# OSUrobotics/KinovaGrasping

Measured on AMD Instinct MI355X. Metric: env-steps/sec (whole node) at 4096 envs/GPU, higher is better.
Workload: dtype f32

## Files before the change

### include/kinova_sim.h

```cpp
#ifndef KINOVA_SIM_H
#define KINOVA_SIM_H
#include <stddef.h>
#include <stdint.h>

#ifdef __cplusplus
extern "C" {
#endif

#define KS_NQ 16
#define KS_NV 15
#define KS_NACT 4
#define KS_NOBS 82
#define KS_NINFO 3
#define KS_NCON_MAX 24
#define KS_NCON_MAX_MG 40
#define KS_CONTACT_STRIDE 20

typedef enum {
    KS_OK = 0,
    KS_ERR_INVALID = -1,
    KS_ERR_NO_DEVICE = -2,
    KS_ERR_HIP = -3,
    KS_ERR_MODEL = -4,
    KS_ERR_STATE = -5
// ... 49 lines not shown
int ks_set_env_params(ks_ctx *ctx, const void *obj_mass, const void *obj_mu, void *stream);

int ks_set_param_ranges(ks_ctx *ctx, const void *ranges, uint64_t seed, void *stream);
int ks_get_env_params(ks_ctx *ctx, void *mass, void *mu, int64_t *episode, void *stream);

int ks_substep(ks_ctx *ctx, const void *ctrl, void *stream);

int ks_obs_from_snapshot(ks_ctx *ctx, const void *snap, const void *rays, void *obs, void *reward, uint8_t *done, void *info, void *stream);

typedef struct {
    const float *actor_pub;
    const int64_t *actor_ver;
    int64_t actor_stride;
    int64_t off_w1, off_b1, off_w2, off_b2, off_w3, off_b3;
    int32_t h1, h2;
    float sigma, max_action;
    int32_t skip_steps;
    int32_t with_replay;
    uint64_t seed;
    float *obs, *prev_obs;
    uint8_t *has_prev, *ready, *lifting;
    int64_t *t, *steps_total;
    float *action, *action_t;
    float *reward_out; uint8_t *done_out;
    void *sim_obs, *sim_reward; uint8_t *sim_done; void *sim_info, *sim_final_obs;
    int32_t horizon, n_steps;
    float *cur_state, *cur_next, *cur_action, *cur_reward, *cur_not_done;
    int64_t *cur_len;
    uint8_t *cur_sel;
    int64_t *pub_len;
    int64_t *counters;
    int64_t budget_ticks;
    int64_t *repeats;
} ks_rollout_args;
int ks_rollout(ks_ctx *ctx, int32_t n_iter, const ks_rollout_args *args_host, void *stream);

enum { KS_CONTROLLER_NONE = 0, KS_CONTROLLER_NAIVE = 1, KS_CONTROLLER_POSITION_DEPENDENT = 2, KS_CONTROLLER_COMBINED = 3 };
enum { KS_LIFT_RULE_TRAIN = 0, KS_LIFT_RULE_EXPERT = 1 };
int ks_set_rollout_controller(ks_ctx *ctx, int32_t mode, int32_t lift_rule, void *stream);
int ks_get_rollout_controller(ks_ctx *ctx, int32_t *mode, int32_t *lift_rule, float *init, void *stream);

enum { KS_PLAN_WAVES = 0, KS_PLAN_WORKGROUPS = 1, KS_PLAN_QUEUE = 2, KS_PLAN_RUNS = 3, KS_PLAN_ROUND_ROBIN = 4 };
int ks_rollout_plan(ks_ctx *ctx, int32_t *mode, int32_t *groups, int32_t *workgroups);

int ks_kernel_time(ks_ctx *ctx, int reset, double *avg_ms_host, int64_t *launches_host);

int ks_version(void);

#ifdef __cplusplus
}
#endif
#endif
```

### kinovagrasping_amd/build.py

```python
from __future__ import annotations

import os
import shutil
import subprocess
from pathlib import Path

PKG = Path(__file__).resolve().parent
CSRC = PKG / "csrc"
LIB = PKG / "libkinova_sim.so"
LIB_MG = PKG / "libkinova_sim_mg.so"
SOURCES = ["ks_api.hip", "ks_rollout.hip", "ks_mlp.hip", "ks_xchg.hip"]
HEADERS = ["ks_math.h", "ks_model.h", "ks_model_host.h", "ks_core.h", "ks_obs.h", "ks_env.h", "ks_mlp_tile.h", "../../include/kinova_sim.h", "../../include/kinova_rollout.h"]


def hipcc_path() -> str:
    for cand in (os.environ.get("HIPCC"), shutil.which("hipcc"), "/opt/rocm/bin/hipcc"):
        if cand and Path(cand).exists():
            return cand
    raise RuntimeError("hipcc not found (need ROCm; this package has no CPU build)")


def needs_build(lib: Path = LIB) -> bool:
    if not lib.exists():
        return True
    t = lib.stat().st_mtime
    return any((CSRC / f).stat().st_mtime > t for f in SOURCES + HEADERS)


def build(force: bool = False, verbose: bool = False, multi_geom: bool | None = None) -> Path:
    for mg in ([False, True] if multi_geom is None else [bool(multi_geom)]):
        lib = LIB_MG if mg else LIB
        if not force and not needs_build(lib):
            continue
        cmd = [hipcc_path(), "--offload-arch=gfx950", "-O3", "-std=c++17", "-fPIC", "-shared"] + (["-DKS_MULTI_GEOM"] if mg else []) + \
              ["-o", str(lib)] + [str(CSRC / s) for s in SOURCES]
        if verbose:
            cmd.insert(1, "-Rpass-analysis=kernel-resource-usage")
        subprocess.check_call(cmd, cwd=str(CSRC))
    return LIB_MG if multi_geom else LIB
```

### kinovagrasping_amd/csrc/ks_api.hip

```cpp
#include <hip/hip_runtime.h>

#include <algorithm>
#include <cstdio>
#include <cstdlib>
#include <cstring>
#include <type_traits>
#include <map>
#include <string>
#include <vector>

#include "../../include/kinova_sim.h"
#include "ks_env.h"
#include "ks_mlp_tile.h"
#include "ks_select.h"
#include "ks_model_host.h"

using namespace ks;

namespace {

constexpr int WAVE = 64;
thread_local std::string g_create_error;

template <typename T> struct StartPool {
    int32_t k, pad;
    uint64_t seed;
    const T *qpos0, *hand_quat, *obs0;
    T *env_qpos0, *env_hand_quat, *env_obs0;
    int64_t *episode;
    int32_t *index;
};

template <typename T> struct EpisodeLog {
    int32_t capacity, pad;
    unsigned long long *written;
    ks_episode_record *ring;
    int32_t *ordinal;
    const int32_t *obj_id;
    const T *obs0;
    const StartPool<T> *pool;
};

template <typename T> struct ParamRanges {
    int32_t active, pad;
    uint64_t seed;
    const T *ranges;
    T *envp;
// ... 757 lines not shown
    kmlp::f32x4(*H1)[NR] = (kmlp::f32x4(*)[NR])(float*)wblocks;
    kmlp::f32x4(*H2)[NR] = H1 + NT1 * 4;
    kmlp::f32x4(*X)[NR] = H2 + NT2 * 4;
    const int lane = threadIdx.x & 63;
    for (;;) {
        const long long ver = uniform64(__hip_atomic_load(ra.actor_ver, __ATOMIC_RELAXED, __HIP_MEMORY_SCOPE_AGENT));
        __builtin_amdgcn_fence(__ATOMIC_ACQUIRE, "agent");
        const float* pw = ra.actor_pub + (ver % 3) * ra.actor_stride;
        kmlp::f32x4 z4 = {0.f, 0.f, 0.f, 0.f};
        int ln = lane, rw = row_env;
        asm volatile("" : "+v"(ln), "+v"(rw));
        const bool mine = kmlp::mlp3_rows_wave<NT1, NT2, true, NR>(ln, (long)rw, S, ra.h1, ra.h2, A, ra.obs, S, kmlp::x_bytes(N, 0, S, S), pw + ra.off_w1,
                                                                     pw + ra.off_b1, pw + ra.off_w2, pw + ra.off_b2, pw + ra.off_w3, X, H1, H2, z4);
        float y[4] = {0.f, 0.f, 0.f, 0.f};
        if (mine) policy_squash(ra, z4, pw + ra.off_b3, y);
        __builtin_amdgcn_fence(__ATOMIC_ACQUIRE, "agent");
        const long long ver2 = uniform64(__hip_atomic_load(ra.actor_ver, __ATOMIC_RELAXED, __HIP_MEMORY_SCOPE_AGENT));
        if (ver2 - ver < 2) {
            if (mine) policy_select(ra, N, row_env, y);
            return;
        }
        if (lane == 0 && ra.repeats) atomicAdd((unsigned long long*)ra.repeats, 1ull);
    }
}

#ifdef KS_ROLLOUT_STAMP
#define KS_RS(i) { const long long t1_ = wall_clock64(); if (C::tid() == 0) atomicAdd((unsigned long long*)&rap->counters[4 + i], (unsigned long long)(t1_ - tk)); tk = t1_; }
#else
#define KS_RS(i)
#endif
template <int NT1, int NT2, bool WAVE_SCOPE>
__device__ __forceinline__ void rollout_iter(const Model<float>& m, const Hulls<float>& hu, const Buffers<float>* __restrict__ bdev, int N, int frame_skip,
                                             int iters, int epw, int pair_memory, const ObsOut<float>* __restrict__ out,
                                             const ks_rollout_args* __restrict__ rap, KS_LDS float* blocks, int grp) {
    using T = float;
    using C = Crew<WAVE_SCOPE>;
    const Buffers<T>& b = *bdev;
    const int e = threadIdx.x / LANE_STRIDE;
    const Team<SUBS> team{(int)threadIdx.x % LANE_STRIDE};
    const int env = e < epw ? b.slot_env[grp * epw + e] : -1;
    const bool active = !(team.sub >= SUBS || env < 0);
    const int wave = WAVE_SCOPE ? (int)(threadIdx.x >> 6) : 0;
    const int slot0 = grp * epw + 4 * wave, cepw = WAVE_SCOPE ? (epw - 4 * wave < 4 ? (epw - 4 * wave < 0 ? 0 : epw - 4 * wave) : 4) : epw;
    KS_LDS T* cblocks = blocks + 4 * wave * SCR_TOTAL;
    KS_LDS unsigned* w = (KS_LDS unsigned*)cblocks;
    const auto join = [] {
        if constexpr (!WAVE_SCOPE) __threadfence_block();
        C::sync();
    };
#ifdef KS_ROLLOUT_STAMP
    long long tk = wall_clock64();
#endif
    {
        const int nn = C::tid() & 15;
        const int row_env = nn < cepw ? b.slot_env[slot0 + nn] : -1;
        if (b.ctl->mode != 0) rollout_controller(b.ctl, rap, N, C::tid() < 16 ? row_env : -1);
        else if constexpr (WAVE_SCOPE) rollout_policy_wave<NT1, NT2>(rap, N, row_env, cblocks);
        else rollout_policy<NT1, NT2>(rap, N, row_env, cblocks);
    }
    join();
    KS_RS(0)
    if (active) {
        T hq[4], act[4];
        KS_UNROLL
        for (int i = 0; i < 4; i++) { hq[i] = b.hand_quat[(long)i * N + env]; act[i] = rap->action_t[(long)i * N + env]; }
        int ncon = 0, status = 0;
        ColW<T> snap{b.snap + env, N};
        KS_LDS T* blk = blocks + e * SCR_TOTAL;
        ScratchC<T, KS_LDS T*> scr{blk};
        T* stp = (T*)(blk + SCR_STATE);
        load_state_team<T, SUBS>(b, env, N, stp, team.sub);
        load_env_params(scr, team, b, env, N);
        constexpr int WPL = (NPAIR_MAX + SUBS - 1) / SUBS;
        PairWarm gw[WPL];
        unsigned* pm = b.pairmem + ((long)env * SUBS + team.sub) * (WPL * WARM_WORDS);
        KS_UNROLL
// ... 25 lines not shown
    if (active) rollout_store<float>(rap, N, env, team.sub);
    join();
    KS_RS(3)
}
#undef KS_RS

struct GroupDeal {
    int n, g0, g1, gstep;
    __device__ __forceinline__ explicit GroupDeal(int n_groups) {
        const bool rr = n_groups < 0;
        n = rr ? -n_groups : n_groups;
        g0 = rr ? (int)blockIdx.x : (int)((long)blockIdx.x * n / gridDim.x);
        g1 = rr ? n : (int)((long)(blockIdx.x + 1) * n / gridDim.x);
        gstep = rr ? (int)gridDim.x : 1;
    }
    __device__ __forceinline__ bool several() const { return g1 - g0 > gstep; }
};
__device__ __forceinline__ bool object_differs(const int32_t* wg_model, int grp, int& staged) {
    const int want = __builtin_amdgcn_readfirstlane(wg_model[grp]);
    if (want == staged) return false;
    staged = want;
    return true;
}

__device__ __noinline__ int rollout_restage(const Model<float>* __restrict__ mp, KS_LDS float* lds0, Hulls<float>* hup) {
    __syncthreads();
    const Model<float>* ml = stage_model_and_tables<float, WG>(mp, lds0);
    int hull_words = 0;
    __syncthreads();
    stage_hulls<float, true>(*ml, lds0 + model_words<float>(), hull_words, *hup, true);
    return (hull_words >> 2) << 2;
}

template <int NT1, int NT2>
__global__ __launch_bounds__(WG) KS_ROLLOUT_REGS void k_rollout(const Model<float>* __restrict__ models, Buffers<float> b, const Buffers<float>* __restrict__ bdev, int N,
                                                int frame_skip, int iters, int epw, int pair_memory, const ObsOut<float>* __restrict__ out,
                                                const ks_rollout_args* __restrict__ rap, int n_iter, int n_groups, int* __restrict__ queue, int wave_free) {
    using T = float;
    extern __shared__ __attribute__((aligned(16))) unsigned char smem[];
#ifdef KS_ROLLOUT_STAMP
    const long long wk_entry = wall_clock64();
#endif
    const GroupDeal deal(n_groups);
    KS_LDS T* const lds0 = (KS_LDS T*)smem;
    KS_LDS T* const lds = lds0 + model_words<T>();
    Hulls<T>* const hup = (Hulls<T>*)(smem + (sizeof(Model<T>) + 15) / 16 * 16);
    int staged = __builtin_amdgcn_readfirstlane(b.wg_model[deal.g0]);
    const Model<T>* ml = stage_model_and_tables<T, WG>(models + staged, lds0);
    int hull_words = 0;
    __syncthreads();
    stage_hulls<T, true>(*ml, lds, hull_words, *hup, true);
    KS_LDS T* blocks = env_blocks(lds, hull_words);
#ifdef KS_ROLLOUT_STAMP
    const long long wk_loop = wall_clock64();
    const long long ck_loop = clock64();
#endif
#define KS_STEP_GROUP(WAVE_SCOPE, GRP)                                                                                      \
    const Model<T>* mi = ml;                                                                                                \
    Hulls<T>* hi = hup;                                                                                                     \
    const Buffers<T>* bi = bdev;                                                                                            \
    const ObsOut<T>* oi = out;                                                                                              \
    const ks_rollout_args* ri = rap;                                                                                        \
    KS_LDS T* ki = blocks;                                                                                                  \
    int gi = GRP;                                                                                                           \
    asm volatile("" : "+s"(mi), "+s"(hi), "+s"(bi), "+s"(oi), "+s"(ri), "+s"(gi));                                          \
    asm volatile("" : "+v"(ki));                                                                                            \
    rollout_iter<NT1, NT2, WAVE_SCOPE>(*mi, *hi, bi, N, frame_skip, iters, epw, pair_memory, oi, ri, ki, gi)
    if (wave_free) {
        const long long budget = rap->budget_ticks, t_end = wall_clock64() + budget;
#pragma clang loop unroll(disable)
        for (int it = 0; it < n_iter; it++) {
            if (budget > 0 && it > 0 && wall_clock64() - t_end > 0) break;
            KS_STEP_GROUP(true, deal.g0);
        }
        return;
    }
    if (queue != nullptr) {
        __shared__ int s_grp;
        int* const q_head = queue, * const q_tail = queue + 1, * const q_steps = queue + ROLLOUT_Q_STEPS;
        unsigned* const ring = (unsigned*)(queue + ROLLOUT_Q_RING);
        const int total = deal.n * n_iter;
#pragma clang loop unroll(disable)
        for (;;) {
            __syncthreads();
            if (threadIdx.x == 0) {
                const int t = atomicAdd(q_head, 1);
                int grp = -1;
                if (t < total) {
                    const unsigned lap = (unsigned)(t / ROLLOUT_QCAP) + 1u;
                    unsigned v = __hip_atomic_load(&ring[t % ROLLOUT_QCAP], __ATOMIC_ACQUIRE, __HIP_MEMORY_SCOPE_AGENT);
                    while ((v >> 12) != lap) {
                        __builtin_amdgcn_s_sleep(16);
                        v = __hip_atomic_load(&ring[t % ROLLOUT_QCAP], __ATOMIC_ACQUIRE, __HIP_MEMORY_SCOPE_AGENT);
                    }
                    grp = (int)(v & 4095u) - 1;
                }
                s_grp = grp;
            }
            __syncthreads();
            const int grp = __builtin_amdgcn_readfirstlane(s_grp);
            if (grp < 0) break;
            __builtin_amdgcn_fence(__ATOMIC_ACQUIRE, "agent");
            if (object_differs(bdev->wg_model, grp, staged)) blocks = lds + rollout_restage(models + staged, lds0, hup);
            KS_STEP_GROUP(false, grp);
            __builtin_amdgcn_fence(__ATOMIC_RELEASE, "agent");
            __syncthreads();
            if (threadIdx.x == 0) {
                const int c = q_steps[gi] + 1;
                q_steps[gi] = c;
                if (c < n_iter) {
                    __builtin_amdgcn_fence(__ATOMIC_RELEASE, "agent");
                    const int t2 = atomicAdd(q_tail, 1);
                    __hip_atomic_store(&ring[t2 % ROLLOUT_QCAP], (((unsigned)(t2 / ROLLOUT_QCAP) + 1u) << 12) | (unsigned)(gi + 1), __ATOMIC_RELEASE, __HIP_MEMORY_SCOPE_AGENT);
                }
            }
        }
        return;
    }
#pragma clang loop unroll(disable)
    for (int it = 0; it < n_iter; it++) {
#pragma clang loop unroll(disable)
        for (int grp = deal.g0; grp < deal.g1; grp += deal.gstep) {
            if (deal.several() && object_differs(bdev->wg_model, grp, staged)) blocks = lds + rollout_restage(models + staged, lds0, hup);
            KS_STEP_GROUP(false, grp);
        }
    }
#undef KS_STEP_GROUP
#ifdef KS_ROLLOUT_STAMP
    if (threadIdx.x == 0 && blockIdx.x < 512) {
        const long long wk_end = wall_clock64();
        rap->counters[8 + blockIdx.x] = wk_entry;
        rap->counters[8 + 512 + blockIdx.x] = wk_loop - wk_entry;
        rap->counters[8 + 1024 + blockIdx.x] = wk_end - wk_loop;
        rap->counters[8 + 1536 + blockIdx.x] = clock64() - ck_loop;
    }
#endif
}

template <typename T, bool USE_LDS>
__global__ __launch_bounds__(WG) void k_substep(const Model<T>* __restrict__ models, Buffers<T> b, const T* __restrict__ ctrl, int N, int iters, int epw, int tap) {
    extern __shared__ __attribute__((aligned(16))) unsigned char smem[];
    KS_LDS T* lds = (KS_LDS T*)smem;
    const Model<T>* mp = models + b.wg_model[blockIdx.x];
    const Model<T>* ml = mp;
    if constexpr (USE_LDS) { ml = stage_model(mp, lds); lds += model_words<T>(); }
    const Model<T>& m = *ml;
    int hull_words = 0;
    static_assert(sizeof(Hulls<T>) <= HULLS_BYTES, "Hulls descriptor slot");
    Hulls<T> hu_own;
    Hulls<T>* hup = &hu_own;
    if constexpr (USE_LDS) hup = (Hulls<T>*)(smem + (sizeof(Model<T>) + 15) / 16 * 16);
    stage_hulls<T, USE_LDS>(*mp, lds, hull_words, *hup);
    const Hulls<T>& hu = *hup;
    const int e = threadIdx.x / LANE_STRIDE;
    const Team<SUBS> team{(int)threadIdx.x % LANE_STRIDE};
    const int env = e < epw ? b.slot_env[blockIdx.x * epw + e] : -1;
    if (team.sub >= SUBS || env < 0) return;
// ... 766 lines not shown
        HIPCHK(hipMemcpy(d_model, table.data(), sizeof(Model<T>) * nm, hipMemcpyHostToDevice));
        if ((r = alloc(&b.nominal, nominal.size()))) return r;
        HIPCHK(hipMemcpy(b.nominal, nominal.data(), nominal.size() * sizeof(T), hipMemcpyHostToDevice));
        {
            std::vector<T> ep(2 * (size_t)cfg.n_envs, nominal[1]);
            std::fill(ep.begin(), ep.begin() + cfg.n_envs, nominal[0]);
            HIPCHK(hipMemcpy(b.envp, ep.data(), ep.size() * sizeof(T), hipMemcpyHostToDevice));
        }
        if ((r = plan_launch()) != KS_OK) return r;
        n_wg = (cfg.n_envs + lpw - 1) / lpw + (nm - 1);
        if ((r = alloc(&b.slot_env, (size_t)n_wg * lpw))) return r;
        if ((r = alloc(&b.wg_model, (size_t)n_wg))) return r;
        if ((r = alloc(&b.n_used, (size_t)1))) return r;
        if ((r = alloc(&b.rayq, (size_t)4 + 2 * (size_t)n_wg))) return r;
        if (obs_in_step && cfg.frame_skip >= 1 && !(getenv("KS_RAY_POOL") && getenv("KS_RAY_POOL")[0] == '0')) {
            ray_pool = 2;
        }
        if ((r = regroup(0, true))) return r;
        if ((r = alloc(&d_b, (size_t)1))) return r;
        if ((r = alloc(&d_out, (size_t)1))) return r;
        if (!h_out) HIPCHK(hipHostMalloc((void**)&h_out, (H_OUT_RING + CAPTURE_RECORDS) * sizeof(ObsOut<T>), hipHostMallocDefault));
        if (!d_ra) HIPCHK(hipMalloc((void**)&d_ra, sizeof(ks_rollout_args)));
        if (!d_queue) HIPCHK(hipMalloc((void**)&d_queue, ROLLOUT_Q_WORDS * sizeof(int)));
        if (!h_ra) HIPCHK(hipHostMalloc((void**)&h_ra, sizeof(ks_rollout_args) * (H_OUT_RING + CAPTURE_RECORDS), hipHostMallocDefault));
        HIPCHK(hipMemcpy(d_b, &b, sizeof b, hipMemcpyHostToDevice));
        model_loaded = true;
        return KS_OK;
    }
    int blocks() const { return (cfg.n_envs + WAVE - 1) / WAVE; }
    int resident_wgs = 256;
    int* d_queue = nullptr;
    bool rollout_queue = !MULTI_GEOM;
    bool rollout_waves = !(getenv("KS_ROLLOUT_WAVES") && getenv("KS_ROLLOUT_WAVES")[0] == '0');
    int rollout_phase_deal = getenv("KS_ROLLOUT_PHASE_DEAL") ? atoi(getenv("KS_ROLLOUT_PHASE_DEAL")) : 1;
    bool rollout_round_robin = false;
    int lpw = WAVE;
    bool rays_in_step = false, obs_in_step = false;
    int ray_pool = 0;
    size_t step_lds = 0;
    int hull_words = 0;
    int plan_launch() {
        {
            int cus = 0;
            if (hipDeviceGetAttribute(&cus, hipDeviceAttributeMultiprocessorCount, device) != hipSuccess || cus <= 0) cus = 256;
            if (const char* e = getenv("KS_ROLLOUT_WGS")) { const int v = atoi(e); if (v > 0) cus = v; }
            resident_wgs = cus;
            rollout_round_robin = n_models > 1;
            if (const char* e = getenv("KS_ROLLOUT_DEAL")) { rollout_round_robin = strcmp(e, "rr") == 0; rollout_queue = strcmp(e, "queue") == 0; }
        }
        const size_t lds_max = 160 * 1024;
        const size_t hull_bytes = (size_t)hull_words * sizeof(T) + (USE_LDS ? (size_t)model_words<T>() * sizeof(T) : 0);
        const size_t per_env = USE_LDS ? (size_t)SCR_TOTAL * sizeof(T) : 0;
        int cap = USE_LDS ? (int)((lds_max - hull_bytes - 64) / per_env) : EPW_MAX;
        if (cap > EPW_MAX) cap = EPW_MAX;
        if (cap < 1) { error = "hull tables do not fit in LDS"; return KS_ERR_MODEL; }
        int want = cfg.envs_per_wave > 0 ? cfg.envs_per_wave : EPW_MAX;
        lpw = want > cap ? cap : want;
        step_lds = hull_bytes + per_env * lpw;
        rays_in_step = USE_LDS && sizeof(T) == 4 && (size_t)wg_rays_words(lpw) <= (size_t)SCR_TOTAL * lpw &&
                       !(getenv("KS_RAYS_IN_STEP") && getenv("KS_RAYS_IN_STEP")[0] == '0');
        obs_in_step = rays_in_step && (size_t)(wg_rays_words(EPW_MAX) + wg_obs_words(EPW_MAX) + 4) <= (size_t)SCR_TOTAL * lpw &&
                      !(getenv("KS_OBS_IN_STEP") && getenv("KS_OBS_IN_STEP")[0] == '0');
        if (getenv("KS_DEBUG")) fprintf(stderr, "[ks] stepping kernel: %d envs per workgroup, LDS %zu B (tables %zu B, %zu B per env), limit %zu\n", lpw, step_lds, hull_bytes, per_env, lds_max);
        HIPCHK(hipFuncSetAttribute((const void*)step_kernel(), hipFuncAttributeMaxDynamicSharedMemorySize, (int)step_lds));
        HIPCHK(hipFuncSetAttribute((const void*)k_substep<T, USE_LDS>, hipFuncAttributeMaxDynamicSharedMemorySize, (int)step_lds));
        return KS_OK;
    }
    static constexpr auto step_kernel() {
        if constexpr (sizeof(T) == 4) return &k_env_step_f32;
        else return &k_env_step<T, USE_LDS>;
    }
    ObsOut<T> out_record(void* obs, void* reward, uint8_t* done, void* info, void* final_obs) const {
        return ObsOut<T>{(T*)obs, (T*)reward, done, (T*)info, (T*)final_obs, cfg.horizon, cfg.auto_reset, cfg.obs_env_major};
    }
    int regroup(hipStream_t s, bool loading = false) {
        hipLaunchKernelGGL(k_slots, dim3(1), dim3(SLOT_THREADS), 0, s, b.obj_id, cfg.n_envs, n_models, lpw, n_wg, b.slot_env, b.wg_model, b.n_used);
        if (loading) {
            HIPCHK(hipGetLastError());
            HIPCHK(hipDeviceSynchronize());
        } else if (stream_is_capturing(s)) { n_groups = n_wg; return KS_OK; }
        HIPCHK(hipMemcpyAsync(&n_groups, b.n_used, sizeof(int32_t), hipMemcpyDeviceToHost, s));
        HIPCHK(hipStreamSynchronize(s));
        return KS_OK;
    }
    void clear_pool(hipStream_t s) {
// ... 140 lines not shown
                                  lpw, (const ObsOut<T>*)d_out, (const ks_rollout_args*)d_ra, n_iter, rollout_round_robin ? -n_groups : n_groups,
                                  (int)ws_offset);
        });
#endif
    }
    int rollout(int n_iter, const ks_rollout_args* ra, hipStream_t s) override {
        if (int r = need_model("ks_rollout")) return r;
        if constexpr (sizeof(T) != 4) return rollout_exact(n_iter, ra, s);
        else {
            int r;
            if ((r = check_rollout_buffers(n_iter, ra))) return r;
            if (!obs_in_step || !cfg.obs_env_major || !cfg.auto_reset) { error = "ks_rollout needs the in-kernel observation path, env-major observations and auto_reset"; return KS_ERR_STATE; }
            if ((r = check_rollout_actor(ra))) return r;
            if (policy_lds_bytes(ra->h1, ra->h2) > (size_t)SCR_TOTAL * lpw * sizeof(T)) { error = "ks_rollout: no LDS for the policy"; return KS_ERR_STATE; }
            const int N = cfg.n_envs;
            const bool wave_free = plan_waves() && policy_wave_lds_bytes(ra->h1, ra->h2) <= (size_t)SCR_TOTAL * 4 * sizeof(T);
            if (ra->budget_ticks != 0 && (ra->budget_ticks < 0 || !wave_free)) {
                error = "ks_rollout: a time budget needs the wave form of the rollout kernel (ks_rollout_plan: KS_PLAN_WAVES)";
                return KS_ERR_STATE;
            }
            if ((r = send_rollout_records(ra, s))) return r;
            const bool use_queue = plan_queue();
            if (use_queue) {
                hipLaunchKernelGGL(k_rollout_queue_init, dim3(1), dim3(256), 0, s, d_queue, n_groups);
            }
            if (wave_free && rollout_phase_deal != 0 && n_models == 1 && ra->budget_ticks == 0) {
                if (rollout_phase_deal == 2 && N <= PHASE_ENVS_MAX) hipLaunchKernelGGL(k_slots_by_phase, dim3(1), dim3(PHASE_THREADS), 0, s, (const int64_t*)ra->t, N, n_wg * lpw, b.slot_env);
                else if (lpw <= 16) hipLaunchKernelGGL(k_slots_by_phase_in_groups, dim3((n_groups + 255) / 256), dim3(256), 0, s, (const int64_t*)ra->t, n_groups, lpw, b.slot_env);
            }
            return launch_for_widths(ra, [&](auto tiles) {
                using W = decltype(tiles);
                return launch_rollout(k_rollout<W::NT1, W::NT2>, step_lds, s, d_model, b, (const Buffers<T>*)d_b, N, cfg.frame_skip, cfg.solver_iterations, lpw,
                                      (int)cfg.pair_memory, (const ObsOut<T>*)d_out, (const ks_rollout_args*)d_ra, n_iter,
                                      (use_queue || !rollout_round_robin) ? n_groups : -n_groups, use_queue ? d_queue : (int*)nullptr, (int)wave_free);
            });
        }
    }
    bool plan_queue() const { return rollout_queue && n_groups > resident_wgs && n_groups <= ROLLOUT_QCAP; }
    bool plan_waves() const {
        return rollout_waves && !plan_queue() && n_groups <= resident_wgs && lpw == EPW_MAX && LANE_STRIDE == SUBS &&
               (size_t)(wg_rays_words(4, WAVE) + wg_obs_words(4) + 4) <= (size_t)SCR_TOTAL * 4;
    }
    int rollout_plan(int32_t* mode, int32_t* groups, int32_t* workgroups) override {
        if (int r = need_model("ks_rollout_plan")) return r;
        if constexpr (sizeof(T) != 4) {
            if (mode) *mode = n_groups <= resident_wgs ? KS_PLAN_WORKGROUPS : (rollout_round_robin ? KS_PLAN_ROUND_ROBIN : KS_PLAN_RUNS);
        } else if (mode) *mode = plan_waves() ? KS_PLAN_WAVES : (n_groups <= resident_wgs ? KS_PLAN_WORKGROUPS : (plan_queue() ? KS_PLAN_QUEUE : (rollout_round_robin ? KS_PLAN_ROUND_ROBIN : KS_PLAN_RUNS)));
        if (groups) *groups = n_groups;
        if (workgroups) *workgroups = n_groups < resident_wgs ? n_groups : resident_wgs;
        return KS_OK;
    }
    int set_start_pool(int k, const void* q0, const void* hq, uint64_t seed, void* obs, hipStream_t s) override {
        if (int r = need_model("ks_set_start_pool")) return r;
        if (k == 0) {
            clear_pool(s);
            HIPCHK(hipGetLastError());
            return KS_OK;
        }
        if (k < 1 || k > POOL_K_MAX || !q0 || !hq) { error = "ks_set_start_pool: 1 <= k <= 1024 starts per env (0 clears the pool), qpos0 and hand_quat required"; return KS_ERR_INVALID; }
        const size_t N = cfg.n_envs;
        int r;
        if (!pb.snap) {
            Buffers<T> t = b;
            if ((r = alloc(&t.qpos, NQ * N))) return r;
            if ((r = alloc(&t.qvel, NV * N))) return r;
            if ((r = alloc(&t.warm, NV * N))) return r;
            if ((r = alloc(&t.rays, NRAY * N))) return r;
// ... 312 lines not shown
```

### kinovagrasping_amd/pipeline.py

```python
from __future__ import annotations

import os
from functools import partial

import torch


def _concurrent_stream(main, dev, tries=8):
    import time
    import warnings
    torch.cuda.synchronize(dev)
    e0, e1 = torch.cuda.Event(enable_timing=True), torch.cuda.Event(enable_timing=True)
    with torch.cuda.stream(main):
        e0.record(main)
        torch.cuda._sleep(1000000)
        e1.record(main)
    torch.cuda.synchronize(dev)
    ms = max(1e-3, e0.elapsed_time(e1))
    spin = int(1000000 * min(1e4, 25.0 / ms))
    flag = torch.zeros(1, device=dev)
    cand = None
    for _ in range(tries):
        cand = torch.cuda.Stream(dev)
        ev = torch.cuda.Event()
# ... 295 lines not shown
                        for _ in range(self.updates_per_step - 1):
                            self.g_head.replay()
                            self._body()
                main.wait_event(self.head_done)
        elif learn:
            for _ in range(self.updates_per_step):
                self.g_head.replay()
                self._body()
        if self.direct_post:
            self.eng.post(commit=False)
        else:
            self.g_post.replay()
        self.pending_commit = self.defer_commit
        self.steps += 1
        return self.eng.reward_out, self.eng.done_out

    def _commit_pending(self):
        if self.pending_commit:
            self.g_commit.replay()
            self.pending_commit = False

    def flush(self, finish_update=False):
        if self.pending_commit or finish_update:
            self.side.wait_stream(self.main)
            with torch.cuda.stream(self.side):
                self._commit_pending()
                if finish_update:
                    self.native.finish_pending()
            self.main.wait_stream(self.side)
        if self.distributed and self.native.exchange is not None:
            self.native.exchange.check()


def rollout_args(sim, policy, eng, pub, pub_ver, steps_total, counters, replay=None, repeats=None, sigma=None):
    from .rollout import SKIP_NUM_TS
    from .sim import KsRolloutArgs
    P = lambda t: t.data_ptr()
    a = KsRolloutArgs()
    if getattr(eng, "controller", None) is None or policy is not None:
        flat, actor = policy._flat_params["actor"], policy.actor
        off = lambda t: (t.data_ptr() - flat.data_ptr()) // 4
        a.actor_pub, a.actor_ver, a.actor_stride = P(pub), P(pub_ver), pub.shape[1]
        a.off_w1, a.off_b1, a.off_w2, a.off_b2, a.off_w3, a.off_b3 = (off(actor.l1.weight), off(actor.l1.bias), off(actor.l2.weight), off(actor.l2.bias),
                                                                      off(actor.l3.weight), off(actor.l3.bias))
        a.h1, a.h2 = actor.l1.weight.shape[0], actor.l2.weight.shape[0]
    a.sigma, a.max_action, a.skip_steps, a.with_replay, a.seed = (eng.sigma if sigma is None else sigma), eng.max_action, SKIP_NUM_TS, int(replay is not None), eng.noise_seed
    a.obs, a.prev_obs, a.has_prev, a.ready, a.lifting = P(eng.obs), P(eng.prev_obs), P(eng.has_prev), P(eng.ready), P(eng.lifting)
    a.t, a.steps_total, a.action, a.action_t = P(eng.t), P(steps_total), P(eng.action), P(eng.action_t)
    a.reward_out, a.done_out = P(eng.reward_out), P(eng.done_out)
    a.sim_obs, a.sim_reward, a.sim_done, a.sim_info, a.sim_final_obs = P(sim.obs), P(sim.reward), P(sim.done), P(sim.info), P(sim.final_obs)
    if replay is not None:
        a.horizon, a.n_steps = replay.horizon, replay.n_steps
        a.cur_state, a.cur_next, a.cur_action = P(replay.a_state), P(replay.a_next), P(replay.a_action)
        a.cur_reward, a.cur_not_done, a.cur_len = P(replay.a_reward), P(replay.a_not_done), P(replay.a_len)
        a.cur_sel, a.pub_len = P(replay.a_sel), P(replay.pub_len)
    a.counters = P(counters)
    if repeats is not None:
        a.repeats = P(repeats)
    return a


class AsyncTrainer(GraphedTrainer):

    def __init__(self, sim, policy, replay, engine, batch_episodes=64, expert_replay=None, expert_prob=0.3, updates_per_step=1,
                 launch_synchronous=False, max_launch_steps=60, balanced=False, prioritized=False, per_alpha=0.3, per_beta=1.0, per_eps=1e-3,
                 per_eps_expert=1.0, tables=None):
        if prioritized and launch_synchronous:
            raise ValueError("AsyncTrainer: launch_synchronous stages episodes in a ring without priorities - not with prioritized=True")
        super().__init__(sim, policy, replay, engine, batch_episodes=batch_episodes, overlap=True, expert_replay=expert_replay, expert_prob=expert_prob,
                         updates_per_step=updates_per_step, lean_learner="auto", balanced=balanced, prioritized=prioritized, per_alpha=per_alpha,
                         per_beta=per_beta, per_eps=per_eps, per_eps_expert=per_eps_expert, tables=tables)
        self.launch_synchronous = bool(launch_synchronous)
        if self.launch_synchronous and getattr(replay, "ep_class", None) is not None:
            raise ValueError("AsyncTrainer: launch_synchronous stages episodes in a ring without classes - not with a replay that has classes set")
        if self.launch_synchronous:
            from .replay import DeviceEpisodeReplay
            self.stage = DeviceEpisodeReplay(replay.n_envs, capacity=(max(1, int(max_launch_steps)) // 10 + 2) * replay.n_envs, horizon=replay.horizon, state_dim=replay.ep_state.shape[2],
                                             action_dim=replay.ep_action.shape[2], n_steps=replay.n_steps, device=replay.device)
            self._stage_rank = torch.zeros(self.stage.capacity, dtype=torch.long, device=replay.device)
            self._stage_pos = torch.arange(1, self.stage.capacity + 1, dtype=torch.long, device=replay.device)
            g = torch.Generator(device="cpu").manual_seed(0)
            self._key_w = (torch.rand(replay.horizon * replay.ep_action.shape[2], generator=g, dtype=torch.float64).to(replay.device),
                           torch.rand(replay.ep_state.shape[2], generator=g, dtype=torch.float64).to(replay.device))
        eng, dev = engine, self.dev
        if not self.native.lds_free:
            raise ValueError("AsyncTrainer needs the LDS-free learner kernels (hidden widths 256-256 / 128-128 / 64-64, or the lean ones: 400-300): the persistent rollout kernel "
                             "holds every CU's LDS for the whole launch, a learner built on library GEMMs could only run behind it")
        self.replica_sync = "per-update" if self.distributed else "single rank"
        self.library_allreduce_chunk = None
        if self.distributed and self.native.exchange is None:
            import torch.distributed as dist
            forced = os.environ.get("KS_ASYNC_SYNC", "")
            if forced == "average":
                import warnings
                warnings.warn("AsyncTrainer: KS_ASYNC_SYNC=average - replicas apply LOCAL updates and are averaged at every launch boundary (periodic model "
                              "averaging), not north_star's per-update gradient all-reduce", RuntimeWarning)
                self.replica_sync = "average-per-launch"
                self.native.local_gradients = True
                self.exchange_note += "; free-running rollout kept: local updates, replicas averaged at every launch boundary"
            elif dist.get_backend(policy.process_group) == "nccl":
                self.library_allreduce_chunk = int(os.environ.get("KS_ASYNC_LIBRARY_CHUNK", "6"))
                self.exchange_note += (f"; no peer mapping: per-update library all-reduce, which executes between launches - keep launches at <= "
                                       f"{self.library_allreduce_chunk} env-steps (the learner lags by at most one launch)")
        if not (eng.native and eng.device_noise and eng._fused_actor_layers() is not None and sim.cfg.auto_reset and sim.obs_env_major):
            raise ValueError("AsyncTrainer needs the fused actor path (3-layer MLP at a supported width, in-kernel noise), auto_reset and env-major obs")
        flat = policy.acting_flat()
        self.actor_flat = flat
        stride = (flat.numel() + 3) // 4 * 4
        self.pub = torch.zeros(3, stride, device=dev)
        self.pub_ver = torch.zeros(1, dtype=torch.long, device=dev)
        self.n_pub = 0
        self.pub[0, :flat.numel()].copy_(flat)
        replay.enable_async()
        self.steps_total = torch.zeros(eng.n, dtype=torch.long, device=dev)
        self.counters = torch.zeros(8 + 4 * 512 + 8 + (eng.n if os.environ.get("KS_DEBUG_DROPS") else 0), dtype=torch.long, device=dev)
        self.repeats = torch.zeros(1, dtype=torch.long, device=dev)
        a = rollout_args(sim, policy, eng, self.pub, self.pub_ver, self.steps_total, self.counters, replay=replay, repeats=self.repeats)
        from .sim import load_library
        self._lib = load_library()
        self.check_in_body = False
        self.pace_lead = int(os.environ.get("KS_ASYNC_LEAD", "8"))
        self.pace_timeouts = torch.zeros(1, dtype=torch.long, device=dev)
        self.args = a
        self.env_steps = 0
        self.rollout_plan, n_groups, n_wgs = sim.rollout_plan()
        self.groups_per_workgroup = (n_groups + n_wgs - 1) // n_wgs
        if self.rollout_plan in ("runs", "round-robin") and n_groups % n_wgs:
            import warnings
            warnings.warn(f"AsyncTrainer: {n_groups} env groups dealt to {n_wgs} persistent workgroups ({self.rollout_plan}): some step {self.groups_per_workgroup} groups per "
                          f"env-step, others {self.groups_per_workgroup - 1} - the launch runs at the pace of the former (the ready queue, KS_ROLLOUT_DEAL=queue, and "
                          "GraphedTrainer's lock-step launches balance such a batch dynamically)", RuntimeWarning)

    def _stage_published(self):
        self.replay.commit_published(into=self.stage)

    def _launch_boundary(self):
        self.g_boundary.replay()
        self.publish()

    def _boundary_commit(self):
        r, st_ = self.replay, self.stage
        self._stage_published()
        cap = st_.capacity
        valid = torch.arange(cap, device=st_.device) < st_._count
        key = (st_.ep_action[:cap].reshape(cap, -1).double() * self._key_w[0]).sum(1) + (st_.ep_state[:cap, 0].double() * self._key_w[1]).sum(1) \
            + st_.ep_len[:cap].double() * 1e-3
        key = torch.where(valid, key, torch.full_like(key, float("inf")))
        order = torch.sort(key, stable=True).indices
        self._stage_rank.scatter_(0, order, self._stage_pos)
        skip = (st_._count - r.capacity).clamp(min=0)
# ... 119 lines not shown
        bufs = [pol._flat_params[k] for k in self._network_names()]
        bufs += [b for net in self._opt_nets() for b in (net.exp_avg, net.exp_avg_sq)]
        flat = torch.cat([b.reshape(-1) for b in bufs])
        dist.all_reduce(flat, op=dist.ReduceOp.SUM, group=pol.process_group)
        flat.div_(world)
        off = 0
        for b in bufs:
            b.copy_(flat[off:off + b.numel()].view_as(b))
            off += b.numel()
        if not self.launch_synchronous:
            self.publish()

    def step(self):
        self.run(1)
        return self.eng.reward_out, self.eng.done_out

    def flush(self, finish_update=False):
        self.side.wait_stream(self.main)
        with torch.cuda.stream(self.side):
            if self.launch_synchronous:
                self._launch_boundary()
            else:
                self.g_commit.replay() if self.g_commit is not None else self.replay.commit_published()
            if finish_update:
                self.native.finish_pending()
                self.publish()
        self.main.wait_stream(self.side)
        if self.distributed and self.native.exchange is not None:
            self.native.exchange.check()

    def repeated_forwards(self) -> int:
        return int(self.repeats.item())

    def counts(self):
        c = self.counters[:4].tolist()
        return {"episodes_finished": c[0], "lifted": c[1], "episodes_kept": c[2], "episodes_dropped": c[3], "pacing_timeouts": int(self.pace_timeouts.item())}
```

### kinovagrasping_amd/sim.py

```python
from __future__ import annotations

import ctypes as C
from pathlib import Path

import torch

from . import build as _build

NQ, NV, NACT, NOBS, NINFO, NCON_MAX, CONTACT_STRIDE = 16, 15, 4, 82, 3, 24, 20
NCON_MAX_MG = 40
SOLVER_ITERATIONS = 20
ASSETS = Path(__file__).resolve().parent / "assets"


class KsConfig(C.Structure):
    _fields_ = [("n_envs", C.c_int32), ("frame_skip", C.c_int32), ("horizon", C.c_int32), ("solver_iterations", C.c_int32),
                ("precision", C.c_int32), ("auto_reset", C.c_int32), ("obs_env_major", C.c_int32), ("envs_per_wave", C.c_int32),
                ("contact_tap", C.c_int32), ("pair_memory", C.c_int32), ("reserved", C.c_int32 * 2)]


class KrRing(C.Structure):
    _fields_ = [("count", C.c_void_p), ("head", C.c_void_p), ("capacity", C.c_int32), ("ep_len", C.c_void_p), ("ep_state", C.c_void_p),
                ("ep_next", C.c_void_p), ("ep_action", C.c_void_p), ("ep_reward", C.c_void_p), ("ep_not_done", C.c_void_p)]


class KsRolloutArgs(C.Structure):
    _fields_ = ([("actor_pub", C.c_void_p), ("actor_ver", C.c_void_p), ("actor_stride", C.c_int64)] +
                [(k, C.c_int64) for k in ("off_w1", "off_b1", "off_w2", "off_b2", "off_w3", "off_b3")] +
                [("h1", C.c_int32), ("h2", C.c_int32), ("sigma", C.c_float), ("max_action", C.c_float), ("skip_steps", C.c_int32),
                 ("with_replay", C.c_int32), ("seed", C.c_uint64)] +
                [(k, C.c_void_p) for k in ("obs", "prev_obs", "has_prev", "ready", "lifting", "t", "steps_total", "action", "action_t", "reward_out",
                                           "done_out", "sim_obs", "sim_reward", "sim_done", "sim_info", "sim_final_obs")] +
                [("horizon", C.c_int32), ("n_steps", C.c_int32)] +
                [(k, C.c_void_p) for k in ("cur_state", "cur_next", "cur_action", "cur_reward", "cur_not_done", "cur_len", "cur_sel", "pub_len", "counters")] +
                [("budget_ticks", C.c_int64), ("repeats", C.c_void_p)])


class KsEpisodeRecord(C.Structure):
    _fields_ = [("env", C.c_int32), ("object", C.c_int32), ("start_index", C.c_int32), ("steps", C.c_int32), ("done", C.c_int32),
                ("start_x", C.c_float), ("start_y", C.c_float), ("episode", C.c_int32)]


EPISODE_RECORD_WORDS = 8
CONTROLLER_MODES = {None: 0, "naive": 1, "position-dependent": 2, "combined": 3}
LIFT_RULES = {"train": 0, "expert": 1}


def controller_codes(mode, lift_rule):
    if mode not in CONTROLLER_MODES or lift_rule not in LIFT_RULES:
        raise ValueError(f"controller {mode!r} / lift rule {lift_rule!r}: one of {[m for m in CONTROLLER_MODES if m]} (or None) and one of {list(LIFT_RULES)}")
    return CONTROLLER_MODES[mode], LIFT_RULES[lift_rule]

EPISODE_LOG_CAPACITY_MAX = 1 << 24


def decode_episode_ring(ring: torch.Tensor, written: int, cursor: int, capacity: int):
    written, cursor, capacity = int(written), int(cursor), int(capacity)
    if tuple(ring.shape) != (capacity, EPISODE_RECORD_WORDS) or ring.dtype != torch.int32:
        raise ValueError("decode_episode_ring: ring int32 [capacity, 8]")
    if not 0 <= cursor <= written:
        raise ValueError("decode_episode_ring: 0 <= cursor <= written")
    first = max(cursor, written - capacity)
    tickets = torch.arange(first, written, dtype=torch.long, device=ring.device)
    return ring[tickets % capacity], first - cursor


def episode_records(words: torch.Tensor) -> dict:
    words = words.contiguous()
# ... 389 lines not shown
```

Before: 2.938 million.

## Add intra-workgroup wave work-stealing takeover for wave-free rollout

Adds an LDS-based protocol that lets a wave that has finished its own iterations request half of another wave's env slots in the same workgroup and keep stepping them. The aim is to cut idle tail time when waves in a workgroup finish unevenly, keeping CUs busy until all env slots finish their iterations. In exchange each iteration adds a small state-machine step with LDS atomics, a noinline call and possible spin-sleeps. It runs by default when the budget is zero, and adds takeover counters to the rollout args.

```diff
diff --git a/include/kinova_sim.h b/include/kinova_sim.h
--- a/include/kinova_sim.h
+++ b/include/kinova_sim.h
@@ -105,6 +105,7 @@
     int64_t *counters;
     int64_t budget_ticks;
     int64_t *repeats;
+    int64_t *takeovers;
 } ks_rollout_args;
 int ks_rollout(ks_ctx *ctx, int32_t n_iter, const ks_rollout_args *args_host, void *stream);
 
diff --git a/kinovagrasping_amd/build.py b/kinovagrasping_amd/build.py
--- a/kinovagrasping_amd/build.py
+++ b/kinovagrasping_amd/build.py
@@ -10,7 +10,7 @@
 LIB = PKG / "libkinova_sim.so"
 LIB_MG = PKG / "libkinova_sim_mg.so"
 SOURCES = ["ks_api.hip", "ks_rollout.hip", "ks_mlp.hip", "ks_xchg.hip"]
-HEADERS = ["ks_math.h", "ks_model.h", "ks_model_host.h", "ks_core.h", "ks_obs.h", "ks_env.h", "ks_mlp_tile.h", "../../include/kinova_sim.h", "../../include/kinova_rollout.h"]
+HEADERS = ["ks_math.h", "ks_model.h", "ks_model_host.h", "ks_core.h", "ks_obs.h", "ks_env.h", "ks_mlp_tile.h", "ks_select.h", "ks_controller.h", "ks_takeover.h", "../../include/kinova_sim.h", "../../include/kinova_rollout.h"]
 
 
 def hipcc_path() -> str:
diff --git a/kinovagrasping_amd/csrc/ks_api.hip b/kinovagrasping_amd/csrc/ks_api.hip
--- a/kinovagrasping_amd/csrc/ks_api.hip
+++ b/kinovagrasping_amd/csrc/ks_api.hip
@@ -13,6 +13,7 @@
 #include "ks_env.h"
 #include "ks_mlp_tile.h"
 #include "ks_select.h"
+#include "ks_takeover.h"
 #include "ks_model_host.h"
 
 using namespace ks;
@@ -836,16 +837,17 @@
 template <int NT1, int NT2, bool WAVE_SCOPE>
 __device__ __forceinline__ void rollout_iter(const Model<float>& m, const Hulls<float>& hu, const Buffers<float>* __restrict__ bdev, int N, int frame_skip,
                                              int iters, int epw, int pair_memory, const ObsOut<float>* __restrict__ out,
-                                             const ks_rollout_args* __restrict__ rap, KS_LDS float* blocks, int grp) {
+                                             const ks_rollout_args* __restrict__ rap, KS_LDS float* blocks, int grp, int sbase, int cnt) {
     using T = float;
     using C = Crew<WAVE_SCOPE>;
     const Buffers<T>& b = *bdev;
     const int e = threadIdx.x / LANE_STRIDE;
     const Team<SUBS> team{(int)threadIdx.x % LANE_STRIDE};
-    const int env = e < epw ? b.slot_env[grp * epw + e] : -1;
+    const int wteam = (int)(threadIdx.x & (WAVE - 1)) >> 4;
+    const int env = WAVE_SCOPE ? (wteam < cnt ? b.slot_env[sbase + wteam] : -1) : (e < epw ? b.slot_env[grp * epw + e] : -1);
     const bool active = !(team.sub >= SUBS || env < 0);
     const int wave = WAVE_SCOPE ? (int)(threadIdx.x >> 6) : 0;
-    const int slot0 = grp * epw + 4 * wave, cepw = WAVE_SCOPE ? (epw - 4 * wave < 4 ? (epw - 4 * wave < 0 ? 0 : epw - 4 * wave) : 4) : epw;
+    const int slot0 = WAVE_SCOPE ? sbase : grp * epw, cepw = WAVE_SCOPE ? cnt : epw;
     KS_LDS T* cblocks = blocks + 4 * wave * SCR_TOTAL;
     KS_LDS unsigned* w = (KS_LDS unsigned*)cblocks;
     const auto join = [] {
@@ -937,6 +939,38 @@
     return (hull_words >> 2) << 2;
 }
 
+struct TakeoverLds {
+    KS_LDS uint32_t* w;
+    __device__ __forceinline__ uint32_t load(int i) { return __hip_atomic_load(w + i, __ATOMIC_RELAXED, __HIP_MEMORY_SCOPE_WORKGROUP); }
+    __device__ __forceinline__ void store(int i, uint32_t v) { __hip_atomic_store(w + i, v, __ATOMIC_RELAXED, __HIP_MEMORY_SCOPE_WORKGROUP); }
+    __device__ __forceinline__ bool cas(int i, uint32_t expect, uint32_t v) {
+        return __hip_atomic_compare_exchange_strong(w + i, &expect, v, __ATOMIC_RELAXED, __ATOMIC_RELAXED, __HIP_MEMORY_SCOPE_WORKGROUP);
+    }
+    __device__ __forceinline__ void release() { __builtin_amdgcn_fence(__ATOMIC_RELEASE, "agent"); }
+    __device__ __forceinline__ void acquire() { __builtin_amdgcn_fence(__ATOMIC_ACQUIRE, "agent"); }
+    __device__ __forceinline__ int64_t deadline_ticks() const { return 5000000; }
+};
+__device__ __noinline__ uint32_t rollout_takeover_next(uint32_t run, KS_LDS uint32_t* words, const ks_rollout_args* __restrict__ rap) {
+    uint32_t next = 0u;
+    if ((threadIdx.x & (WAVE - 1)) == 0) {
+        TakeoverLds mem{words};
+        kstk::Wave w = kstk::resume((int)(threadIdx.x >> 6), run);
+        for (;;) {
+            w.idle = 0;
+            const kstk::Event ev = kstk::advance(w, mem, (int64_t)wall_clock64());
+            if (ev == kstk::STEP) { next = kstk::pack_run(w.off, w.cnt, w.left); break; }
+            if (ev == kstk::EXIT) break;
+            if (w.idle) __builtin_amdgcn_s_sleep(64);
+        }
+        if (int64_t* tk = rap->takeovers) {
+            if (w.grants) atomicAdd((unsigned long long*)&tk[0], (unsigned long long)w.grants);
+            if (w.expiries) atomicAdd((unsigned long long*)&tk[1], (unsigned long long)w.expiries);
+            if (w.grants_from_pairs) atomicAdd((unsigned long long*)&tk[2], (unsigned long long)w.grants_from_pairs);
+        }
+    }
+    return (uint32_t)__builtin_amdgcn_readfirstlane((int)next);
+}
+
 template <int NT1, int NT2>
 __global__ __launch_bounds__(WG) KS_ROLLOUT_REGS void k_rollout(const Model<float>* __restrict__ models, Buffers<float> b, const Buffers<float>* __restrict__ bdev, int N,
                                                 int frame_skip, int iters, int epw, int pair_memory, const ObsOut<float>* __restrict__ out,
@@ -953,6 +987,8 @@
     int staged = __builtin_amdgcn_readfirstlane(b.wg_model[deal.g0]);
     const Model<T>* ml = stage_model_and_tables<T, WG>(models + staged, lds0);
     int hull_words = 0;
+    __shared__ uint32_t s_tko[kstk::WORDS];
+    if (wave_free == 2 && threadIdx.x < kstk::WORDS) s_tko[threadIdx.x] = kstk::initial_word((int)threadIdx.x, epw, n_iter);
     __syncthreads();
     stage_hulls<T, true>(*ml, lds, hull_words, *hup, true);
     KS_LDS T* blocks = env_blocks(lds, hull_words);
@@ -960,23 +996,28 @@
     const long long wk_loop = wall_clock64();
     const long long ck_loop = clock64();
 #endif
-#define KS_STEP_GROUP(WAVE_SCOPE, GRP)                                                                                      \
+#define KS_STEP_GROUP(WAVE_SCOPE, GRP, SBASE, CNT)                                                                          \
     const Model<T>* mi = ml;                                                                                                \
     Hulls<T>* hi = hup;                                                                                                     \
     const Buffers<T>* bi = bdev;                                                                                            \
     const ObsOut<T>* oi = out;                                                                                              \
     const ks_rollout_args* ri = rap;                                                                                        \
     KS_LDS T* ki = blocks;                                                                                                  \
-    int gi = GRP;                                                                                                           \
-    asm volatile("" : "+s"(mi), "+s"(hi), "+s"(bi), "+s"(oi), "+s"(ri), "+s"(gi));                                          \
+    int gi = GRP, si = SBASE, ci = CNT;                                                                                     \
+    asm volatile("" : "+s"(mi), "+s"(hi), "+s"(bi), "+s"(oi), "+s"(ri), "+s"(gi), "+s"(si), "+s"(ci));                      \
     asm volatile("" : "+v"(ki));                                                                                            \
-    rollout_iter<NT1, NT2, WAVE_SCOPE>(*mi, *hi, bi, N, frame_skip, iters, epw, pair_memory, oi, ri, ki, gi)
+    rollout_iter<NT1, NT2, WAVE_SCOPE>(*mi, *hi, bi, N, frame_skip, iters, epw, pair_memory, oi, ri, ki, gi, si, ci)
     if (wave_free) {
         const long long budget = rap->budget_ticks, t_end = wall_clock64() + budget;
+        const int wave = __builtin_amdgcn_readfirstlane((int)(threadIdx.x >> 6));
+        uint32_t run = kstk::pack_run(4 * wave, kstk::initial_cnt(wave, epw), wave_free == 2 ? n_iter + 1 : n_iter);
 #pragma clang loop unroll(disable)
-        for (int it = 0; it < n_iter; it++) {
-            if (budget > 0 && it > 0 && wall_clock64() - t_end > 0) break;
-            KS_STEP_GROUP(true, deal.g0);
+        for (int it = 0;; it++) {
+            if (wave_free == 2) {
+                run = (uint32_t)__builtin_amdgcn_readfirstlane((int)rollout_takeover_next(run, (KS_LDS uint32_t*)s_tko, rap));
+                if (run == 0u) break;
+            } else if (it >= n_iter || (budget > 0 && it > 0 && wall_clock64() - t_end > 0)) break;
+            KS_STEP_GROUP(true, deal.g0, __builtin_amdgcn_readfirstlane(deal.g0 * epw + kstk::run_off(run)), __builtin_amdgcn_readfirstlane(kstk::run_cnt(run)));
         }
         return;
     }
@@ -1007,7 +1048,7 @@
             if (grp < 0) break;
             __builtin_amdgcn_fence(__ATOMIC_ACQUIRE, "agent");
             if (object_differs(bdev->wg_model, grp, staged)) blocks = lds + rollout_restage(models + staged, lds0, hup);
-            KS_STEP_GROUP(false, grp);
+            KS_STEP_GROUP(false, grp, 0, 0);
             __builtin_amdgcn_fence(__ATOMIC_RELEASE, "agent");
             __syncthreads();
             if (threadIdx.x == 0) {
@@ -1027,7 +1068,7 @@
 #pragma clang loop unroll(disable)
         for (int grp = deal.g0; grp < deal.g1; grp += deal.gstep) {
             if (deal.several() && object_differs(bdev->wg_model, grp, staged)) blocks = lds + rollout_restage(models + staged, lds0, hup);
-            KS_STEP_GROUP(false, grp);
+            KS_STEP_GROUP(false, grp, 0, 0);
         }
     }
 #undef KS_STEP_GROUP
@@ -1860,6 +1901,7 @@
     int* d_queue = nullptr;
     bool rollout_queue = !MULTI_GEOM;
     bool rollout_waves = !(getenv("KS_ROLLOUT_WAVES") && getenv("KS_ROLLOUT_WAVES")[0] == '0');
+    bool rollout_takeover = !(getenv("KS_ROLLOUT_TAKEOVER") && getenv("KS_ROLLOUT_TAKEOVER")[0] == '0');
     int rollout_phase_deal = getenv("KS_ROLLOUT_PHASE_DEAL") ? atoi(getenv("KS_ROLLOUT_PHASE_DEAL")) : 1;
     bool rollout_round_robin = false;
     int lpw = WAVE;
@@ -1879,6 +1921,7 @@
         const size_t lds_max = 160 * 1024;
         const size_t hull_bytes = (size_t)hull_words * sizeof(T) + (USE_LDS ? (size_t)model_words<T>() * sizeof(T) : 0);
         const size_t per_env = USE_LDS ? (size_t)SCR_TOTAL * sizeof(T) : 0;
+        static_assert(16 + kstk::WORDS * sizeof(uint32_t) <= 64, "k_rollout's static LDS");
         int cap = USE_LDS ? (int)((lds_max - hull_bytes - 64) / per_env) : EPW_MAX;
         if (cap > EPW_MAX) cap = EPW_MAX;
         if (cap < 1) { error = "hull tables do not fit in LDS"; return KS_ERR_MODEL; }
@@ -2085,7 +2128,8 @@
                 using W = decltype(tiles);
                 return launch_rollout(k_rollout<W::NT1, W::NT2>, step_lds, s, d_model, b, (const Buffers<T>*)d_b, N, cfg.frame_skip, cfg.solver_iterations, lpw,
                                       (int)cfg.pair_memory, (const ObsOut<T>*)d_out, (const ks_rollout_args*)d_ra, n_iter,
-                                      (use_queue || !rollout_round_robin) ? n_groups : -n_groups, use_queue ? d_queue : (int*)nullptr, (int)wave_free);
+                                      (use_queue || !rollout_round_robin) ? n_groups : -n_groups, use_queue ? d_queue : (int*)nullptr,
+                                      wave_free ? ((rollout_takeover && ra->budget_ticks == 0 && n_iter < kstk::LEFT_MAX) ? 2 : 1) : 0);
             });
         }
     }
diff --git a/kinovagrasping_amd/csrc/ks_takeover.h b/kinovagrasping_amd/csrc/ks_takeover.h
--- /dev/null
+++ b/kinovagrasping_amd/csrc/ks_takeover.h
@@ -0,0 +1,154 @@
+#pragma once
+#if defined(__HIPCC__)
+#include <hip/hip_runtime.h>
+#define KTK_HD __host__ __device__ __forceinline__
+#else
+#define KTK_HD inline
+#endif
+#include <stdint.h>
+
+#ifndef KS_TAKEOVER_MIN_LEFT
+#define KS_TAKEOVER_MIN_LEFT 2
+#endif
+
+namespace kstk {
+
+constexpr int WAVES = 4, MIN_LEFT = KS_TAKEOVER_MIN_LEFT;
+constexpr int REQ = 0, PROG = WAVES, GRANT = 2 * WAVES, WORDS = 3 * WAVES;
+constexpr int LEFT_MAX = (1 << 22) - 1;
+constexpr uint32_t GRANT_BIT = 0x80000000u, DECLINED = 0x40000000u, FROM_PAIR = 0x20000000u;
+
+KTK_HD uint32_t pack_prog(int left, int cnt) { return (uint32_t)left << 3 | (uint32_t)cnt; }
+KTK_HD uint32_t pack_run(int off, int cnt, int left) { return (uint32_t)left << 7 | (uint32_t)off << 3 | (uint32_t)cnt; }
+KTK_HD int run_cnt(uint32_t r) { return (int)(r & 7u); }
+KTK_HD int run_off(uint32_t r) { return (int)(r >> 3 & 15u); }
+KTK_HD int run_left(uint32_t r) { return (int)(r >> 7 & (uint32_t)LEFT_MAX); }
+
+enum State : int {
+    W_ITER_DONE, W_CHECK, W_CLAIM, W_ANSWER, W_PUBLISH,
+    H_START, H_SCAN, H_REQUEST, H_WAIT, H_WAIT_TARGET, H_WITHDRAW, H_WAIT_ANSWER, H_TAKE, EXITED
+};
+enum Event : int { NONE, STEP, EXIT };
+
+struct Wave {
+    int me, state;
+    int off, cnt, left;
+    int q;
+    int target, k;
+    int best, best_left, best_cnt, blocked;
+    uint32_t got, prog;
+    int64_t deadline;
+    int expired;
+    int idle;
+    int grants, grants_from_pairs, expiries;
+};
+
+KTK_HD Wave resume(int me, uint32_t run) {
+    Wave w{};
+    w.me = me; w.off = run_off(run); w.cnt = run_cnt(run); w.left = run_left(run);
+    w.state = W_ITER_DONE;
+    return w;
+}
+KTK_HD int initial_cnt(int w, int epw) { return epw - 4 * w < 4 ? (epw - 4 * w < 0 ? 0 : epw - 4 * w) : 4; }
+KTK_HD uint32_t initial_word(int word, int epw, int n_iter) {
+    return (word >= PROG && word < PROG + WAVES) ? pack_prog(n_iter, initial_cnt(word - PROG, epw)) : 0u;
+}
+
+template <class M>
+KTK_HD Event advance(Wave& w, M& mem, int64_t now) {
+    switch (w.state) {
+    case W_ITER_DONE:
+        w.left--;
+        mem.store(PROG + w.me, pack_prog(w.left, w.cnt));
+        w.state = (w.left > 0 && w.cnt > 0) ? W_CHECK : H_START;
+        return NONE;
+    case W_CHECK:
+        w.q = (int)mem.load(REQ + w.me);
+        if (w.q == 0) { w.state = W_ITER_DONE; return STEP; }
+        w.state = W_CLAIM;
+        return NONE;
+    case W_CLAIM:
+        if (!mem.cas(REQ + w.me, (uint32_t)w.q, 0u)) { w.state = W_ITER_DONE; return STEP; }
+        w.state = W_ANSWER;
+        return NONE;
+    case W_ANSWER:
+        if (w.cnt >= 2 && w.left >= MIN_LEFT) {
+            const int give = w.cnt / 2;
+            mem.release();
+            mem.store(GRANT + w.q - 1, GRANT_BIT | pack_run(w.off + w.cnt - give, give, w.left) | (w.cnt == 2 ? FROM_PAIR : 0u));
+            w.cnt -= give;
+            w.state = W_PUBLISH;
+            return NONE;
+        }
+        mem.store(GRANT + w.q - 1, DECLINED);
+        w.state = W_ITER_DONE;
+        return STEP;
+    case W_PUBLISH:
+        mem.store(PROG + w.me, pack_prog(w.left, w.cnt));
+        w.state = W_ITER_DONE;
+        return STEP;
+    case H_START:
+        w.deadline = now + mem.deadline_ticks();
+        w.k = 0; w.best = -1; w.blocked = 0;
+        w.state = H_SCAN;
+        return NONE;
+    case H_SCAN: {
+        const int s = (w.me + 1 + w.k / 2) % WAVES;
+        if ((w.k & 1) == 0) w.prog = mem.load(PROG + s);
+        else {
+            const int left = (int)(w.prog >> 3), cnt = (int)(w.prog & 7u);
+            const bool pending = mem.load(REQ + s) != 0u;
+            if (cnt >= 2 && left > MIN_LEFT) {
+                if (pending) w.blocked = 1;
+                else if (w.best < 0 || left > w.best_left || (left == w.best_left && (cnt > w.best_cnt || (cnt == w.best_cnt && s < w.best)))) {
+                    w.best = s; w.best_left = left; w.best_cnt = cnt;
+                }
+            }
+        }
+        if (++w.k < 2 * (WAVES - 1)) return NONE;
+        if (w.best >= 0) { w.target = w.best; w.state = H_REQUEST; return NONE; }
+        if (w.blocked && now < w.deadline) { w.k = 0; w.blocked = 0; w.idle = 1; return NONE; }
+        w.state = EXITED;
+        return EXIT;
+    }
+    case H_REQUEST:
+        if (mem.cas(REQ + w.target, 0u, (uint32_t)w.me + 1u)) { w.deadline = now + mem.deadline_ticks(); w.expired = 0; w.state = H_WAIT; }
+        else if (now < w.deadline) { w.k = 0; w.best = -1; w.blocked = 0; w.state = H_SCAN; }
+        else { w.state = EXITED; return EXIT; }
+        return NONE;
+    case H_WAIT:
+        w.got = mem.load(GRANT + w.me);
+        w.state = w.got != 0u ? H_TAKE : H_WAIT_TARGET;
+        return NONE;
+    case H_WAIT_TARGET:
+        if ((mem.load(PROG + w.target) >> 3) == 0u) w.state = H_WITHDRAW;
+        else if (now >= w.deadline) { w.expired = 1; w.state = H_WITHDRAW; }
+        else { w.idle = 1; w.state = H_WAIT; }
+        return NONE;
+    case H_WITHDRAW:
+        if (mem.cas(REQ + w.target, (uint32_t)w.me + 1u, 0u)) {
+            if (w.expired) { w.expiries++; w.state = EXITED; return EXIT; }
+            w.state = H_START;
+        } else w.state = H_WAIT_ANSWER;
+        return NONE;
+    case H_WAIT_ANSWER:
+        w.got = mem.load(GRANT + w.me);
+        if (w.got != 0u) w.state = H_TAKE;
+        else w.idle = 1;
+        return NONE;
+    case H_TAKE:
+        mem.store(GRANT + w.me, 0u);
+        if (w.got & GRANT_BIT) {
+            mem.acquire();
+            w.off = run_off(w.got); w.cnt = run_cnt(w.got); w.left = run_left(w.got);
+            w.grants++;
+            if (w.got & FROM_PAIR) w.grants_from_pairs++;
+            w.state = W_PUBLISH;
+        } else w.state = H_START;
+        return NONE;
+    default:
+        return EXIT;
+    }
+}
+
+}
diff --git a/kinovagrasping_amd/pipeline.py b/kinovagrasping_amd/pipeline.py
--- a/kinovagrasping_amd/pipeline.py
+++ b/kinovagrasping_amd/pipeline.py
@@ -351,7 +351,7 @@
             self.native.exchange.check()
 
 
-def rollout_args(sim, policy, eng, pub, pub_ver, steps_total, counters, replay=None, repeats=None, sigma=None):
+def rollout_args(sim, policy, eng, pub, pub_ver, steps_total, counters, replay=None, repeats=None, sigma=None, takeovers=None):
     from .rollout import SKIP_NUM_TS
     from .sim import KsRolloutArgs
     P = lambda t: t.data_ptr()
@@ -376,6 +376,8 @@
     a.counters = P(counters)
     if repeats is not None:
         a.repeats = P(repeats)
+    if takeovers is not None:
+        a.takeovers = P(takeovers)
     return a
 
 
@@ -432,9 +434,10 @@
         self.pub[0, :flat.numel()].copy_(flat)
         replay.enable_async()
         self.steps_total = torch.zeros(eng.n, dtype=torch.long, device=dev)
-        self.counters = torch.zeros(8 + 4 * 512 + 8 + (eng.n if os.environ.get("KS_DEBUG_DROPS") else 0), dtype=torch.long, device=dev)
+        self.counters = torch.zeros(8 + 4 * 512 + 8 + (eng.n if os.environ.get("KS_DEBUG_DROPS") else 0) + 3, dtype=torch.long, device=dev)
         self.repeats = torch.zeros(1, dtype=torch.long, device=dev)
-        a = rollout_args(sim, policy, eng, self.pub, self.pub_ver, self.steps_total, self.counters, replay=replay, repeats=self.repeats)
+        a = rollout_args(sim, policy, eng, self.pub, self.pub_ver, self.steps_total, self.counters, replay=replay, repeats=self.repeats,
+                         takeovers=self.counters[-3:])
         from .sim import load_library
         self._lib = load_library()
         self.check_in_body = False
@@ -620,6 +623,9 @@
     def repeated_forwards(self) -> int:
         return int(self.repeats.item())
 
+    def takeovers(self):
+        return tuple(self.counters[-3:].tolist())
+
     def counts(self):
         c = self.counters[:4].tolist()
         return {"episodes_finished": c[0], "lifted": c[1], "episodes_kept": c[2], "episodes_dropped": c[3], "pacing_timeouts": int(self.pace_timeouts.item())}
diff --git a/kinovagrasping_amd/sim.py b/kinovagrasping_amd/sim.py
--- a/kinovagrasping_amd/sim.py
+++ b/kinovagrasping_amd/sim.py
@@ -33,7 +33,7 @@
                                            "done_out", "sim_obs", "sim_reward", "sim_done", "sim_info", "sim_final_obs")] +
                 [("horizon", C.c_int32), ("n_steps", C.c_int32)] +
                 [(k, C.c_void_p) for k in ("cur_state", "cur_next", "cur_action", "cur_reward", "cur_not_done", "cur_len", "cur_sel", "pub_len", "counters")] +
-                [("budget_ticks", C.c_int64), ("repeats", C.c_void_p)])
+                [("budget_ticks", C.c_int64), ("repeats", C.c_void_p), ("takeovers", C.c_void_p)])
 
 
 class KsEpisodeRecord(C.Structure):
```

New measurement: 3.014 million, median of 6. +2.6%, better.
